# eltoto1219/vltk

Measured on AMD Instinct MI355X. Metric: images/sec FRCNN feature extraction, 800x1333 batch, higher is better.
Workload: dtype f16; 1 GPU; configs[1]: ResNet-101-C4 fp16 (the reference has no FPN: SURVEY.md D1), 32 synthetic 800x1333 images per GPU per step, R=300 RPN proposals through the Res5 head, max 100 detections/img, seeded synthetic weights; global_batch=32, parallelism=image-sharded x1, all-gather of output blocks

## Files before the change

include/vltk_hip.h:

```cpp
#ifndef VLTK_HIP_H
#define VLTK_HIP_H

#include <stddef.h>
#include <stdint.h>

#ifdef __cplusplus
extern "C" {
#endif

#define VK_OK 0
#define VK_EINVAL 1
#define VK_ENOTIMPL 2
#define VK_ENONFINITE 3
#define VK_EWEIGHTS 4
#define VK_EHIP 5
#define VK_ENOMEM 6

typedef enum { VK_F32 = 0, VK_F16 = 1, VK_I64 = 2, VK_I32 = 3, VK_BF16 = 4 } vk_dtype;
typedef enum { VK_ACT_NONE = 0, VK_ACT_RELU = 1, VK_ACT_GELU = 2 , VK_ACT_TANH = 3 } vk_act;

#define VK_MAX_ANCHOR_DIM 8
#define VK_MAX_NMS_THRESH 8

typedef struct vk_config {
// ... 139 lines not shown

size_t vk_packed_weight_bytes(int cout, int cin, int kh, int kw, int groups, vk_dtype dt);
int vk_packed_cout(int cout);
int vk_conv_slice_channels(int cin, int groups);
int vk_pack_conv_weight(const float *w_oihw_host, const float *bn_host, const float *bias_host,
                        int cout, int cin, int kh, int kw, int groups, vk_dtype dt,
                        void *w_packed_host, float *bias_packed_host);

int vk_conv2d(const void *x, int N, int H, int W, int cin,
              const void *w_packed, const float *bias_packed, const void *residual,
              void *y, int cout, int ldy, int kh, int kw, int stride, int pad, int dil, int groups,
              int relu, vk_dtype dt, vk_dtype out_dt, void *stream);

#define VK_ROUTE_GENERIC 0
#define VK_ROUTE_RING 1
#define VK_ROUTE_DUO 2
#define VK_ROUTE_WS 3
#define VK_ROUTE_GEMM4 4
#define VK_ROUTE_PANEL 5
#define VK_ROUTE_BLK 6
int vk_conv_route(int N, int H, int W, int cin, int cin2, int has_residual, int fused_mean, int cout, int ldy, int kh, int kw,
                  int stride, int pad, int dil, int groups, int relu, vk_dtype dt, vk_dtype out_dt);
int vk_panel_phase_images(int N, int H, int W, int dil);

int vk_conv1x1_dual(const void *x1, int cin1, const void *x2, int cin2, long M,
                    const void *w_packed, const float *bias_packed, const void *residual,
                    void *y, int cout, int relu, void *stream);

int vk_bottleneck64(const void *x, int N, int H, int W, int cin, int proj,
                    const void *w1_packed, const float *b1_packed, const void *w2_packed, const float *b2_packed,
                    const void *w3_packed, const float *b3_packed, void *y, void *stream);

int vk_fuse_shortcut(int cin, int cin_shortcut, int cout, int stride, vk_dtype dt);
int vk_bottleneck64_eligible(int cin, int cmid, int cout, int stride, int dil, int groups, int proj, int fused_shortcut,
                             long N, int H, int W, vk_dtype dt);

size_t vk_conv1x1_meanpool_workspace_bytes(int N, int HW, int cout);
int vk_conv1x1_meanpool(const void *x, int N, int HW, int cin, const void *w_packed, const float *bias_packed,
                        const void *residual, int cout, int relu, float *out_mean,
                        void *workspace, size_t workspace_bytes, void *stream);


int vk_linear(const void *x, long M, int K, const void *w_packed, const float *bias_packed, const void *residual,
              void *y, int N, int ldy, int act, vk_dtype dt, vk_dtype out_dt, void *stream);
int vk_layernorm(const void *x, int ldx, const float *gamma, const float *beta, void *y, int ldy, int M, int C,
                 float eps, float scale, int accumulate, vk_dtype dt, void *stream);
// ... 142 lines not shown
```

vltk_amd/_lib.py:

```python
import ctypes as C
import os

_HERE = os.path.dirname(os.path.abspath(__file__))
LIB_PATH = os.path.join(_HERE, "libvltk_hip.so")
if os.environ.get("VLTK_AMD_LIB"):
    LIB_PATH = os.environ["VLTK_AMD_LIB"]
elif os.environ.get("VLTK_AMD_ABLATION_LIB") == "1":
    LIB_PATH = LIB_PATH.replace("libvltk_hip.so", "libvltk_hip_ablation.so")

VK_OK, VK_EINVAL, VK_ENOTIMPL, VK_ENONFINITE, VK_EWEIGHTS, VK_EHIP, VK_ENOMEM = range(7)
VK_F32, VK_F16, VK_I64, VK_I32, VK_BF16 = 0, 1, 2, 3, 4
VK_ACT_NONE, VK_ACT_RELU, VK_ACT_GELU, VK_ACT_TANH = 0, 1, 2, 3
VK_ROUTE_GENERIC, VK_ROUTE_RING, VK_ROUTE_DUO, VK_ROUTE_WS, VK_ROUTE_GEMM4, VK_ROUTE_PANEL, VK_ROUTE_BLK = range(7)
VK_ATT_ROUTE_MFMA, VK_ATT_ROUTE_LDS, VK_ATT_ROUTE_TILED, VK_ATT_ROUTE_STREAM = range(4)
VK_MAX_ANCHOR_DIM = 8
VK_MAX_NMS_THRESH = 8
VK_MAX_IGNOREY = 64
VK_SELECT_CLASS_MAX, VK_SELECT_PER_CLASS, VK_SELECT_DETECTIONS = 0, 1, 2
VK_POOLER_ROIPOOL, VK_POOLER_ROIALIGN, VK_POOLER_ROIALIGNV2 = 0, 1, 2

_EXC = {
    VK_EINVAL: ValueError,
    VK_ENOTIMPL: NotImplementedError,
    VK_ENONFINITE: AssertionError,
# ... 67 lines not shown
                              C.POINTER(C.c_int64)]),
    "vk_forward_begin_ignorey": (_I, [_P, _P, _I, _I, _I, _P, _P, C.POINTER(vk_roi_params), C.POINTER(vk_outputs), _P,
                                      C.POINTER(C.c_int64), C.POINTER(vk_ignorey)]),
    "vk_forward_begin_select": (_I, [_P, _P, _I, _I, _I, _P, _P, C.POINTER(vk_select_params), C.POINTER(vk_outputs), _P,
                                     C.POINTER(C.c_int64), C.POINTER(vk_ignorey)]),
    "vk_forward_boxes_begin": (_I, [_P, _P, _I, _I, _I, _P, _P, _P, _I, _P, C.POINTER(vk_outputs), _P, C.POINTER(C.c_int64)]),
    "vk_forward_grid_begin": (_I, [_P, _P, _I, _I, _I, _P, _P, _I, _I, C.POINTER(vk_outputs), _P, C.POINTER(C.c_int64)]),
    "vk_grid_pool": (_I, [_P, _I, _I, _I, _I, _I, _P, _P, _I, _I, _I, _P, _I, _P, _P]),
    "vk_forward_end": (_I, [_P, C.c_int64]),
    "vk_given_boxes_ingest": (_I, [_P, _P, _P, _P, _I, _I, _P, _P, _P, _I, _I, _F, _I, _P, _P]),
    "vk_given_box_outputs": (_I, [_P, _P, _P, _P, _P, _P, _P, _P, _I, _I, _I, C.POINTER(vk_outputs), _P]),
    "vk_get_stage": (_I, [_P, C.c_char_p, C.POINTER(_P), C.POINTER(_I), C.POINTER(C.c_int64), C.POINTER(_I)]),
    "vk_memcpy_d2d": (_I, [_P, _P, _SZ, _P]),
    "vk_enable_stage_timing": (_I, [_P, _I]),
    "vk_get_stage_timing": (_I, [_P, C.POINTER(_F)]),
    "vk_enable_kernel_timing": (_I, [_P, _I]),
    "vk_get_kernel_timing": (_I, [_P, C.POINTER(C.c_int64), C.POINTER(_D), C.POINTER(_D), C.POINTER(_D), _I]),
    "vk_packed_weight_bytes": (_SZ, [_I, _I, _I, _I, _I, _I]),
    "vk_conv_slice_channels": (_I, [_I, _I]),
    "vk_packed_cout": (_I, [_I]),
    "vk_pack_conv_weight": (_I, [_P, _P, _P, _I, _I, _I, _I, _I, _I, _P, _P]),
    "vk_conv_route": (_I, [_I] * 18),
    "vk_panel_phase_images": (_I, [_I, _I, _I, _I]),
    "vk_conv1x1_dual": (_I, [_P, _I, _P, _I, C.c_long, _P, _P, _P, _P, _I, _I, _P]),
    "vk_bottleneck64": (_I, [_P, _I, _I, _I, _I, _I, _P, _P, _P, _P, _P, _P, _P, _P]),
    "vk_fuse_shortcut": (_I, [_I, _I, _I, _I, _I]),
    "vk_bottleneck64_eligible": (_I, [_I, _I, _I, _I, _I, _I, _I, _I, C.c_long, _I, _I, _I]),
    "vk_conv1x1_meanpool_workspace_bytes": (_SZ, [_I, _I, _I]),
    "vk_conv1x1_meanpool": (_I, [_P, _I, _I, _I, _P, _P, _P, _I, _I, _P, _P, _SZ, _P]),
    "vk_linear": (_I, [_P, C.c_long, _I, _P, _P, _P, _P, _I, _I, _I, _I, _I, _P]),
    "vk_layernorm": (_I, [_P, _I, _P, _P, _P, _I, _I, _I, _F, _F, _I, _I, _P]),
    "vk_embed_layernorm": (_I, [_P, _P, _I, _I, _P, _P, _P, _P, _P, _P, _I, _F, _I, _P]),
    "vk_attention": (_I, [_P, _I, _P, _I, _P, _I, _P, _P, _I, _I, _I, _I, _I, _I, _I, _P]),
    "vk_attention_tiled": (_I, [_P, _I, _P, _I, _P, _I, _P, _P, _I, _I, _I, _I, _I, _I, _I, _P]),
    "vk_attention_route": (_I, [_I] * 9),
    "vk_visualbert_embed": (_I, [_P, _P, _P, _P, _I, _I, _I, _I, _P, _I, _P, _I, _P, _P, _I, _P, _P, _I, _P, _P, _P, _I, _F, _I, _P]),
    "vk_vit_patchify": (_I, [_P, _I, _I, _I, _I, _I, _P, _I, _I, _P]),
    "vk_vit_assemble": (_I, [_P, _I, _P, _P, _I, _I, _P, _I, _I, _P]),
    "vk_roi_align": (_I, [_P, _P, _P, _P, _I, _I, _I, _P, _P, _I, _I, _I, _I, _P, _I, _P]),
    "vk_assign_levels": (_I, [_P, _I, _I, _I, _I, _F, _I, _P, _P]),
    "vk_upsample2x_add": (_I, [_P, _P, _P, _I, _I, _I, _I, _I, _I, _I, _P]),
    "vk_subsample2": (_I, [_P, _P, _I, _I, _I, _I, _I, _P]),
    "vk_relu_copy": (_I, [_P, _P, C.c_long, _I, _P]),
    "vk_rpn_multilevel_workspace_bytes": (_SZ, [_I, _I, _I, _I]),
    "vk_rpn_proposals_multilevel": (_I, [_P, _P, _P, _P, _I, _I, _P, _P, _I, _P, _P, _F, _P, _P, _F, _D, _I, _I, _P, _P, _P, _P, _P, _SZ, _P]),
    "vk_rpn_proposals_multilevel_ignorey": (_I, [_P, _P, _P, _P, _I, _I, _P, _P, _I, _P, _P, _F, _P, _P, _F, _D, _I, _I, _P, _P, _P, _P,
# ... 69 lines not shown
```

vltk_amd/csrc/conv3x3_panel.hip:

```cpp
#include <cstdio>
#include <type_traits>
#include <vector>

#include "vk_common.h"

namespace vk {

typedef _Float16 half8 __attribute__((ext_vector_type(8)));
typedef float floatx4 __attribute__((ext_vector_type(4)));
typedef _Float16 half4 __attribute__((ext_vector_type(4)));
typedef unsigned uintx4 __attribute__((ext_vector_type(4)));

struct PanelK {
    const char *x;
    const char *w;
    const float *bias;
    const char *res;
    char *y;
    int H, W, HW, M;
    int cin_bytes, ldy;
    int dil;
    int cstages;
    int wrow_bytes;
    int relu;
// ... 13 lines not shown
    const int W2 = p.W >> 1, Q = p.HW >> 2;
    const int ph = (gb >= Q ? 1 : 0) + (gb >= 2 * Q ? 1 : 0) + (gb >= 3 * Q ? 1 : 0);
    const int q = gb - ph * Q;
    const int qy = (int)(((unsigned)q * p.rcp_w2) >> 16), qx = q - qy * W2;
    return {qy, qx, (2 * qy + (ph >> 1)) * p.W + 2 * qx + (ph & 1)};
}

constexpr int P_NW = 6;
constexpr int P_WSLOT = 256 * 64;

#define VKP_GLDS16(gptr, lptr)                                                                         \
    __builtin_amdgcn_global_load_lds((const __attribute__((address_space(1))) void *)(gptr),          \
                                     (__attribute__((address_space(3))) void *)(lptr), 16, 0, 0)

template <int J, int PP>
constexpr int panel_in_window() {
    int c = 0;
    for (int d = 1; d <= P_NW - 2; ++d) {
        int t = ((J - d) % 9 + 9) % 9;
        if (t < PP) ++c;
    }
    return c;
}
template <int J>
constexpr int last_w_in_window() {
    int c = 0;
    for (int d = 1; d <= P_NW - 2; ++d) {
        int t = J - d;
        if (t < 0 || t + P_NW < 9) ++c;
    }
    return 2 * c;
}

template <int N>
__device__ __forceinline__ void vm_wait() {
    static_assert(N >= 0 && N <= 15, "vmcnt immediate");
    asm volatile("s_waitcnt vmcnt(%0)" ::"n"(N) : "memory");
}

template <int PP, int DBG, int TAG = 0, int MI = 8, int PHASE = 0>
__global__ __launch_bounds__(512, 2) void conv3x3_panel_kernel(PanelK p) {
    extern __shared__ __attribute__((aligned(16))) char smem[];
    static_assert(MI == 8 || MI == 9, "8 or 9 row tiles per wave");
    static_assert(!PHASE || (PP == 4 && MI == 8 && !(DBG & 9)), "the phase form: halo 128 = (W / 2 + 1) * 16 at W = 14, 256-row tiles");
    static_assert(MI == 8 || !(DBG & 8), "the LDS-staged epilogue is written for 128-row halves");
    constexpr int TILE = 2 * MI * 16;
    constexpr int PROWS = PP * 128;
    constexpr int HALO = (PROWS - TILE) / 2;
    constexpr int PBYTES = PROWS * 64;
    constexpr int WBASE = 2 * PBYTES;
    constexpr bool ZROW = PP == 3;
    constexpr int ZOFF = WBASE + P_NW * P_WSLOT;

    int bid = blockIdx.x;
    const int nwg = p.m_tiles * p.n_tiles;
    unsigned long st_k0 = 0;
    if constexpr (DBG & 4) asm volatile("s_memrealtime %0\n\ts_waitcnt lgkmcnt(0)" : "=s"(st_k0)::"memory");
    if constexpr (PP == 3 || PHASE) {
        if (p.tile_ctr && bid >= p.static_tiles) {
            int *mail = reinterpret_cast<int *>(smem + (PHASE ? 0 : 2 * PP * 128 * 64 + P_NW * P_WSLOT + 128));
            if (threadIdx.x == 0) {
                const unsigned v = atomicAdd(p.tile_ctr, 1u);
                if (v == p.ctr_last) *p.tile_ctr = 0u;
                *mail = p.static_tiles + (int)v;
            }
            __syncthreads();
            bid = __builtin_amdgcn_readfirstlane(*mail);
            if constexpr (PHASE) __syncthreads();
            if (bid >= nwg) return;
        }
    }
    const int q = nwg >> 3, r = nwg & 7, xcd = bid & 7;
    const int t_ = (xcd < r ? xcd * (q + 1) : r * (q + 1) + (xcd - r) * q) + (bid >> 3);
    const int n_tile = t_ % p.n_tiles, m_tile = t_ / p.n_tiles;
    const int m0 = m_tile * TILE, n0 = n_tile * 256;

    const int tid = threadIdx.x, lane = tid & 63;
    const int wave = __builtin_amdgcn_readfirstlane(tid >> 6);
    const int wr = wave >> 2, wc = wave & 3;
    const int g = lane >> 4, j = lane & 15;

    unsigned vm0 = 0, vm1 = 0, vm2 = 0;

    const int lrow = lane >> 2;
    const int lchunk = (lane & 3) ^ ((-(lrow >> 2)) & 3);
    const int pm_first = m0 - HALO + wave * 16 + lrow;
    const unsigned wsrc0 = (unsigned)(n0 + wave * 32 + lrow) * (unsigned)p.wrow_bytes + lchunk * 16;
    const unsigned wstep = 16u * p.wrow_bytes;
    int g0 = 0, gb0 = 0;
    if constexpr (PHASE) {
        g0 = (m0 >> 4) / p.HW;
        gb0 = (m0 >> 4) - g0 * p.HW;
    }
    auto blk_of = [&](int off, int &G) -> int {
        int t = gb0 + off;
        G = g0;
        while (t < 0) {
            t += p.HW;
            --G;
        }
        while (t >= p.HW) {
            t -= p.HW;
            ++G;
        }
        if (G < 0) G = 0, t = 0;
        if (G >= p.groups) G = p.groups - 1, t = p.HW - 1;
        return t;
    };
    [[maybe_unused]] unsigned ps_lane = 0, ps_blk[PP] = {};
    if constexpr (PHASE) {
// ... 2 lines not shown
        for (int q2 = 0; q2 < PP; ++q2) {
            int G;
            const int t = blk_of(wave - HALO / 16 + q2 * 8, G);
            ps_blk[q2] = __builtin_amdgcn_readfirstlane((unsigned)(G * 16 * p.HW + phase_blk(p, t).row) * (unsigned)p.cin_bytes);
        }
    }
    auto req_panel = [&](int cs, int piece) {
        if constexpr (PHASE) {
            unsigned pl = ps_lane;
            asm volatile("" : "+v"(pl));
            VKP_GLDS16(p.x + (pl + (ps_blk[piece] + cs * 64)), smem + (cs & 1) * PBYTES + (piece * 8 + wave) * 1024);
            return;
        }
        int pf = pm_first;
        asm volatile("" : "+v"(pf));
        const int m = min(max(pf + piece * 128, 0), p.M - 1);
        const unsigned off = (unsigned)m * (unsigned)p.cin_bytes + cs * 64 + lchunk * 16;
        VKP_GLDS16(p.x + off, smem + (cs & 1) * PBYTES + (piece * 8 + wave) * 1024);
    };
    auto req_w = [&](int slot, int cs, int tap, int i) {
        const unsigned koff = (unsigned)(tap * p.cstages + cs) * 64;
        unsigned wb_ = wsrc0;
        asm volatile("" : "+v"(wb_));
        VKP_GLDS16(p.w + (wb_ + i * wstep + koff), smem + WBASE + slot * P_WSLOT + (wave * 2 + i) * 1024);
    };

    const unsigned lds0 = (unsigned)(unsigned long)(__attribute__((address_space(3))) char *)smem;
    [[maybe_unused]] const unsigned zrow = lds0 + ZOFF;
    if constexpr (ZROW) {
        if (tid < 16) *reinterpret_cast<unsigned *>(smem + ZOFF + tid * 4) = 0u;
        asm volatile("s_waitcnt lgkmcnt(0)" ::: "memory");
    }
    unsigned w_a[2];
#pragma unroll
    for (int par = 0; par < 2; ++par) {
        const int wrow = wc * 64 + (j >> 2) * 8 + par * 4 + (j & 3);
        w_a[par] = lds0 + WBASE + wrow * 64 + ((g ^ ((-(wrow >> 2)) & 3)) << 4);
    }
    const int jbase = HALO + wr * (MI * 16) + j;
    auto x_addr_of = [&](int parity, int tap) -> unsigned {
        const int shift = PHASE ? ((tap / 3 - 1) * (p.W >> 1) + (tap % 3 - 1)) * 16 : ((tap / 3 - 1) * p.W + (tap % 3 - 1)) * p.dil;
        int jb = jbase;
        asm volatile("" : "+v"(jb));
        const int rb = jb + shift;
        return lds0 + parity * PBYTES + (rb << 6) + ((g ^ ((-(rb >> 2)) & 3)) << 4);
    };

// ... 52 lines not shown
        a0_ += so;                                      \
        a1_ += so;                                      \
        VKP_DSR(WF[0], a0_, 0);                         \
        VKP_DSR(WF[1], a1_, 0);                         \
        VKP_DSR(WF[2], a0_, 2048);                      \
        VKP_DSR(WF[3], a1_, 2048);                      \
    } while (0)

    auto tap_mask = [&](auto j_c) -> unsigned {
        constexpr int J = decltype(j_c)::value;
        unsigned tw = J < 3 ? vm0 : (J < 6 ? vm1 : vm2);
        if constexpr (PHASE)
            asm volatile("" : "+s"(tw));
        else
            asm volatile("" : "+v"(tw));
        return tw >> ((J % 3) * 9);
    };
    auto tap_word = [&](auto j_c) -> unsigned {
        constexpr int J = decltype(j_c)::value;
        unsigned tw = J < 3 ? vm0 : (J < 6 ? vm1 : vm2);
        asm volatile("" : "+v"(tw));
        return tw;
    };
    auto pre = [&](auto last_c, auto odd_c, auto j_c, unsigned xa, unsigned &xa_next, const half8 (&wcur)[4]) {
        constexpr bool LAST = decltype(last_c)::value;
        constexpr int ODD = decltype(odd_c)::value;
        constexpr int J = decltype(j_c)::value;
        const unsigned tm = ZROW ? 0u : tap_mask(j_c);
        [[maybe_unused]] const unsigned tw = ZROW ? tap_word(j_c) : 0u;
        constexpr bool has_next = !(LAST && J == 8);
        if constexpr (has_next) xa_next = (J == 8) ? x_addr_of(1 - ODD, 0) : x_addr_of(ODD, J + 1);
        VKP_DSRX(xw[3], xa, 3072, tw, J, 3); VKP_WAIT3(xw[0]); VKP_SB(); VKP_MMA_ROW(0, xw[0], wcur, tm); VKP_SB();
        VKP_DSRX(xw[0], xa, 4096, tw, J, 4); VKP_WAIT3(xw[1]); VKP_SB(); VKP_MMA_ROW(1, xw[1], wcur, tm); VKP_SB();
        VKP_DSRX(xw[1], xa, 5120, tw, J, 5); VKP_WAIT3(xw[2]); VKP_SB(); VKP_MMA_ROW(2, xw[2], wcur, tm); VKP_SB();
        VKP_DSRX(xw[2], xa, 6144, tw, J, 6); VKP_WAIT3(xw[3]); VKP_SB(); VKP_MMA_ROW(3, xw[3], wcur, tm); VKP_SB();
        if constexpr (MI == 9) {
            VKP_DSRX(xw[3], xa, 7168, tw, J, 7); VKP_DSRX(xw[4], xa, 8192, tw, J, 8); VKP_WAIT4(xw[0]); VKP_SB(); VKP_MMA_ROW(4, xw[0], wcur, tm); VKP_SB();
            asm volatile("s_waitcnt lgkmcnt(0)" : "+v"(xw[1]), "+v"(xw[2]), "+v"(xw[3]), "+v"(xw[MI == 9 ? 4 : 3])::"memory");
        } else {
            VKP_DSRX(xw[3], xa, 7168, tw, J, 7); VKP_WAIT3(xw[0]); VKP_SB(); VKP_MMA_ROW(4, xw[0], wcur, tm); VKP_SB();
            asm volatile("s_waitcnt lgkmcnt(0)" : "+v"(xw[1]), "+v"(xw[2]), "+v"(xw[3])::"memory");
        }
        VKP_SB();
        if constexpr (has_next) {
            constexpr int OUT = LAST ? last_w_in_window<J>() : 2 * (P_NW - 2) + panel_in_window<J, PP>();
            vm_wait<OUT>();
            if constexpr (!(DBG & 48) || ((DBG & 16) && J % 3 == 2)) asm volatile("s_barrier" ::: "memory");
        }
        VKP_SB();
    };
    auto post = [&](auto last_c, auto odd_c, auto j_c, int cs, unsigned xa_next, const half8 (&wcur)[4], half8 (&wnext)[4]) {
        constexpr bool LAST = decltype(last_c)::value;
        constexpr int ODD = decltype(odd_c)::value;
        constexpr int J = decltype(j_c)::value;
        static_assert(!(LAST && J == 8), "the final step has no POST");
        constexpr int SLOT = (3 * ODD + J) % P_NW;
        const unsigned tm = ZROW ? 0u : tap_mask(j_c);
        constexpr int JN = (J + 1) % 9;
        [[maybe_unused]] const unsigned twn = ZROW ? tap_word(std::integral_constant<int, JN>{}) : 0u;
        constexpr bool issue_w = !LAST || (J + P_NW < 9);
        constexpr bool issue_p = !LAST && (J < PP);
        constexpr unsigned so = (unsigned)((SLOT + 1) % P_NW) * P_WSLOT;
        VKP_READ_W(wnext, so);
        VKP_DSRX(xw[0], xa_next, 0, twn, JN, 0);
        VKP_SB();
        VKP_MMA_ROW(5, xw[1], wcur, tm);
        VKP_SB();
        if constexpr (issue_p) req_panel(cs + 1, J);
        if constexpr (issue_w) req_w(SLOT, cs + (J + P_NW) / 9, (J + P_NW) % 9, 0);
        VKP_DSRX(xw[1], xa_next, 1024, twn, JN, 1);
        VKP_SB();
        VKP_MMA_ROW(6, xw[2], wcur, tm);
        VKP_SB();
        if constexpr (issue_w) req_w(SLOT, cs + (J + P_NW) / 9, (J + P_NW) % 9, 1);
        VKP_DSRX(xw[2], xa_next, 2048, twn, JN, 2);
        VKP_SB();
        VKP_MMA_ROW(7, xw[3], wcur, tm);
        VKP_SB();
        if constexpr (MI == 9) {
            VKP_MMA_ROW(8, xw[MI == 9 ? 4 : 3], wcur, tm);
            VKP_SB();
        }
    };
    auto wset = [&](auto u_c) -> half8(&)[4] {
        if constexpr (decltype(u_c)::value % 2 == 0)
            return wa;
        else
            return wb;
    };
#define VKP_IC(V) std::integral_constant<int, (V)> {}
#define VKP_UNIT(LP, LC, U)                                                                                          \
    post(LP, VKP_IC(((U) - 1) / 9), VKP_IC(((U) - 1) % 9), cs + ((U) - 1) / 9, xan, wset(VKP_IC((U) - 1)), wset(VKP_IC(U)));  \
    xa = xan;                                                                                                        \
    pre(LC, VKP_IC((U) / 9), VKP_IC((U) % 9), xa, xan, wset(VKP_IC(U)));
    using T_ = std::integral_constant<bool, true>;
    using F_ = std::integral_constant<bool, false>;

#pragma unroll
    for (int q2 = 0; q2 < PP; ++q2) req_panel(0, q2);
#pragma unroll
    for (int st = 0; st < P_NW; ++st) {
        req_w(st, 0, st, 0);
        req_w(st, 0, st, 1);
    }
    if constexpr (PHASE) {
        unsigned u0 = 0, u1 = 0, u2 = 0;
#pragma unroll
        for (int mi = 0; mi < MI; ++mi) {
            int G;
            const PhaseBlk b = phase_blk(p, blk_of(wr * MI + mi, G));
            const unsigned c0 = b.qx >= 1, c2 = b.qx + 1 < (p.W >> 1);
            const unsigned cw = m0 + (wr * MI + mi) * 16 < p.M ? (c0 << mi) | (1u << (9 + mi)) | (c2 << (18 + mi)) : 0u;
            u0 |= b.qy >= 1 ? cw : 0u;
            u1 |= cw;
            u2 |= b.qy + 1 < (p.H >> 1) ? cw : 0u;
        }
        vm0 = __builtin_amdgcn_readfirstlane(u0);
        vm1 = __builtin_amdgcn_readfirstlane(u1);
        vm2 = __builtin_amdgcn_readfirstlane(u2);
    } else if (p.HW >= MI * 16 + p.W) {
        const int mbase = m0 + wr * (MI * 16);
        const int rem0 = mbase % p.HW, ho0 = rem0 / p.W, wo0 = rem0 - ho0 * p.W;
        const float rcpw = 1.0f / (float)p.W;
#pragma unroll
        for (int mi = 0; mi < MI; ++mi) {
            const int xcol = wo0 + mi * 16 + j;
// ... 17 lines not shown
    } else {
#pragma unroll
        for (int mi = 0; mi < MI; ++mi) {
            const int m = m0 + wr * (MI * 16) + mi * 16 + j;
            if (m < p.M) {
                const int n_img = m / p.HW;
                const int rem = m - n_img * p.HW;
                const int ho = rem / p.W, wo = rem - ho * p.W;
#pragma unroll
                for (int tap = 0; tap < 9; ++tap) {
                    const int hi = ho + (tap / 3 - 1) * p.dil, wi = wo + (tap % 3 - 1) * p.dil;
                    const unsigned ok = ((unsigned)hi < (unsigned)p.H && (unsigned)wi < (unsigned)p.W) ? 1u : 0u;
                    if (tap < 3)
                        vm0 |= ok << (tap * 9 + mi);
                    else if (tap < 6)
                        vm1 |= ok << ((tap - 3) * 9 + mi);
                    else
                        vm2 |= ok << ((tap - 6) * 9 + mi);
                }
            }
        }
    }

    vm_wait<2 * (P_NW - 1)>();
    asm volatile("s_barrier" ::: "memory");
    unsigned long st_c0 = 0, st_r0 = 0;
    if constexpr (DBG & 4) asm volatile("s_memtime %0\n\ts_memrealtime %1\n\ts_waitcnt lgkmcnt(0)" : "=s"(st_c0), "=s"(st_r0)::"memory");
    unsigned xa = x_addr_of(0, 0), xan = 0;
    VKP_READ_W(wa, 0u);
    {
        [[maybe_unused]] const unsigned tw0 = tap_word(VKP_IC(0));
        VKP_DSRX(xw[0], xa, 0, tw0, 0, 0);
        VKP_DSRX(xw[1], xa, 1024, tw0, 0, 1);
        VKP_DSRX(xw[2], xa, 2048, tw0, 0, 2);
    }
    pre(F_{}, VKP_IC(0), VKP_IC(0), xa, xan, wa);
    int cs = 0;
    for (; cs + 2 < CS; cs += 2) {
        VKP_UNIT(F_{}, F_{}, 1) VKP_UNIT(F_{}, F_{}, 2) VKP_UNIT(F_{}, F_{}, 3) VKP_UNIT(F_{}, F_{}, 4) VKP_UNIT(F_{}, F_{}, 5)
        VKP_UNIT(F_{}, F_{}, 6) VKP_UNIT(F_{}, F_{}, 7) VKP_UNIT(F_{}, F_{}, 8) VKP_UNIT(F_{}, F_{}, 9) VKP_UNIT(F_{}, F_{}, 10)
        VKP_UNIT(F_{}, F_{}, 11) VKP_UNIT(F_{}, F_{}, 12) VKP_UNIT(F_{}, F_{}, 13) VKP_UNIT(F_{}, F_{}, 14) VKP_UNIT(F_{}, F_{}, 15)
        VKP_UNIT(F_{}, F_{}, 16) VKP_UNIT(F_{}, F_{}, 17)
        post(F_{}, VKP_IC(1), VKP_IC(8), cs + 1, xan, wb, wa);
        xa = xan;
        pre(F_{}, VKP_IC(0), VKP_IC(0), xa, xan, wa);
    }
    VKP_UNIT(F_{}, F_{}, 1) VKP_UNIT(F_{}, F_{}, 2) VKP_UNIT(F_{}, F_{}, 3) VKP_UNIT(F_{}, F_{}, 4) VKP_UNIT(F_{}, F_{}, 5)
    VKP_UNIT(F_{}, F_{}, 6) VKP_UNIT(F_{}, F_{}, 7) VKP_UNIT(F_{}, F_{}, 8) VKP_UNIT(F_{}, T_{}, 9) VKP_UNIT(T_{}, T_{}, 10)
    VKP_UNIT(T_{}, T_{}, 11) VKP_UNIT(T_{}, T_{}, 12) VKP_UNIT(T_{}, T_{}, 13) VKP_UNIT(T_{}, T_{}, 14) VKP_UNIT(T_{}, T_{}, 15)
    VKP_UNIT(T_{}, T_{}, 16) VKP_UNIT(T_{}, T_{}, 17)
    {
        const unsigned tm = ZROW ? 0u : tap_mask(VKP_IC(8));
        VKP_MMA_ROW(5, xw[1], wb, tm);
        VKP_MMA_ROW(6, xw[2], wb, tm);
        VKP_MMA_ROW(7, xw[3], wb, tm);
        if constexpr (MI == 9) VKP_MMA_ROW(8, xw[MI == 9 ? 4 : 3], wb, tm);
    }
    unsigned long st_c1 = 0, st_r1 = 0;
    if constexpr (DBG & 4) asm volatile("s_memtime %0\n\ts_memrealtime %1\n\ts_waitcnt lgkmcnt(0)" : "=s"(st_c1), "=s"(st_r1)::"memory");
#undef VKP_UNIT
#undef VKP_IC
#undef VKP_DSR
#undef VKP_DSRX
#undef VKP_WAIT3
#undef VKP_WAIT4
#undef VKP_MMA_ROW
#undef VKP_READ_W
#undef VKP_SB
// ... 151 lines not shown
    const long n8 = ((M + 255) / 256 * nt + n_cu - 1) / n_cu, n9 = ((M + 287) / 288 * nt + n_cu - 1) / n_cu;
    if (n8 > 4) return 9;
    return n9 * 9 < n8 * 8 ? 9 : 8;
}

bool conv3x3_panel_eligible(const ConvArgs &a) {
    const char *v = getenv("VK_CONV3X3_PANEL");
    if (v && v[0] == '0') return false;
    if (a.stem || a.dt != VK_F16 || a.out_dt != VK_F16 || a.relu > 1) return false;
    if (a.kh != 3 || a.kw != 3 || a.stride != 1 || a.pad != a.dil) return false;
    if (a.Cout % 256 != 0 || a.ldy != a.Cout || a.Cin % 64 != 0 || a.Cin < 128) return false;
    if (panel_pp(a) == 0) return false;
    if ((long)a.N * a.H * a.W * a.Cin * 2 >= (1L << 32)) return false;
    return true;
}

int conv3x3_panel_phase_images(const ConvArgs &a) {
    const char *v = getenv("VK_PANEL_PHASE");
    if (v && v[0] == '0') return 0;
    if (a.dil != 2 || a.H % 2 != 0 || a.W % 2 != 0 || a.W > 14 || a.H > 1024 || a.N < 16) return 0;
    return a.N / 16 * 16;
}

static int launch_panel_one(const ConvArgs &a, hipStream_t stream, bool phase);

int launch_conv3x3_panel(const ConvArgs &a, hipStream_t stream) {
    const int np = conv3x3_panel_phase_images(a);
    if (np == 0) return launch_panel_one(a, stream, false);
    ConvArgs b = a;
    b.N = np;
    VK_TRY(launch_panel_one(b, stream, true));
    if (np == a.N) return VK_OK;
    const size_t rows = (size_t)np * a.H * a.W;
    b.N = a.N - np;
    b.x = (const char *)a.x + rows * a.Cin * 2;
    b.y = (char *)a.y + rows * a.ldy * 2;
    if (a.res) b.res = (const char *)a.res + rows * a.ldy * 2;
    return launch_panel_one(b, stream, false);
}

static int launch_panel_one(const ConvArgs &a, hipStream_t stream, bool phase) {
    DeviceState *ds = nullptr;
    VK_TRY(device_state(&ds));
    PanelK k;
    k.x = (const char *)a.x;
    k.w = (const char *)a.w;
    k.bias = a.bias;
    k.res = (const char *)a.res;
    k.y = (char *)a.y;
    k.H = a.H;
    k.W = a.W;
    k.HW = a.H * a.W;
    const long M = (long)a.N * a.H * a.W;
    VK_REQUIRE(M > 0 && M < (1L << 31) - 512, VK_EINVAL, "conv3x3_panel: M=%ld out of range", M);
    VK_REQUIRE(M * a.Cin * 2 < (1L << 32) && (long)a.Cout * 9 * a.Cin * 2 < (1L << 32), VK_EINVAL,
               "conv3x3_panel: tensor beyond the 32-bit DMA offsets (M=%ld Cin=%d Cout=%d)", M, a.Cin, a.Cout);
    k.M = (int)M;
    k.cin_bytes = a.Cin * 2;
    k.ldy = a.ldy;
    k.dil = a.dil;
    k.cstages = a.Cin / 32;
    k.wrow_bytes = 9 * a.Cin * 2;
    k.relu = a.relu;
    const int mi = phase ? 8 : panel_mi(a, M, ds->n_cu), pp = phase ? 4 : panel_pp(a, mi);
    k.groups = phase ? a.N / 16 : 0;
    k.rcp_w2 = phase ? 65536u / (unsigned)(a.W / 2) + 1u : 0u;
    k.m_tiles = ceil_div(k.M, mi * 32);
    k.n_tiles = a.Cout / 256;
    Timed t;
    VK_TRY(t.begin(stream));
    const int total_tiles = k.m_tiles * k.n_tiles;
    k.tile_ctr = nullptr;
    k.static_tiles = total_tiles;
    int n_wgs = total_tiles;
    const char *dyn_env = getenv("VK_PANEL_DYNAMIC");
    const bool dyn_off = dyn_env && dyn_env[0] == '0';
    if (!dyn_off && (pp == 3 || phase) && total_tiles >= 16 * 256) {
        VK_TRY(acquire_tile_counter(&k.tile_ctr));
        k.static_tiles = total_tiles * 15 / 16 / 8 * 8;
        n_wgs = total_tiles + (total_tiles / 32 + 63) / 64 * 64;
        k.ctr_last = (unsigned)(n_wgs - k.static_tiles - 1);
    }
    const dim3 grid(n_wgs), block(512);
#ifdef VK_ABLATION
    const int dbg = getenv("VK_CONV256_DBG") ? atoi(getenv("VK_CONV256_DBG")) : 0;
#endif
    const int smem = 2 * pp * 128 * 64 + P_NW * P_WSLOT + (pp == 3 ? 256 : 0);
    k.stamps = nullptr;
#define VKP_LAUNCH(PP_, DBG_, TAG_, MI_)                                                                                                   \
    do {                                                                                                                                   \
        VK_TRY(set_max_lds(conv3x3_panel_kernel<PP_, DBG_, TAG_, MI_>, 2 * PP_ * 128 * 64 + P_NW * P_WSLOT + (PP_ == 3 ? 256 : 0)));        \
        hipLaunchKernelGGL((conv3x3_panel_kernel<PP_, DBG_, TAG_, MI_>), grid, block, smem, stream, k);                                     \
    } while (0)
#ifdef VK_ABLATION
    if (const char *sf = getenv("VK_PANEL_STAMPS"); sf && pp == 3) {
        const size_t nb = (size_t)grid.x * 6 * sizeof(unsigned long);
        VK_CHECK_HIP(hipMalloc((void **)&k.stamps, nb));
        VK_CHECK_HIP(hipMemset(k.stamps, 0, nb));
        if (mi == 9)
            VKP_LAUNCH(3, 4, 0, 9);
        else
            VKP_LAUNCH(3, 4, 0, 8);
        VK_CHECK_HIP(hipStreamSynchronize(stream));
        std::vector<unsigned long> h((size_t)grid.x * 6);
        VK_CHECK_HIP(hipMemcpy(h.data(), k.stamps, nb, hipMemcpyDeviceToHost));
        VK_CHECK_HIP(hipFree(k.stamps));
        if (FILE *f = fopen(sf, "a")) {
            fprintf(f, "# wg k_loop_cycles k_loop_ticks workgroup_ticks ticks_before_k_loop start_tick end_tick (tick = 10 ns)\n");
            for (unsigned w = 0; w < grid.x; ++w)
                fprintf(f, "%u %lu %lu %lu %lu %lu %lu\n", w, h[(size_t)w * 6], h[(size_t)w * 6 + 1], h[(size_t)w * 6 + 2], h[(size_t)w * 6 + 3], h[(size_t)w * 6 + 4],
                        h[(size_t)w * 6 + 5]);
            fclose(f);
        }
    } else if (mi == 8 && pp == 3 && dbg == 8)
        VKP_LAUNCH(3, 8, 0, 8);
    else if (mi == 8 && pp == 3 && dbg == 1)
        VKP_LAUNCH(3, 1, 0, 8);
    else if (mi == 9 && pp == 3 && dbg == 1)
        VKP_LAUNCH(3, 1, 0, 9);
    else if (mi == 9 && pp == 3 && dbg == 16)
        VKP_LAUNCH(3, 16, 0, 9);
    else if (mi == 9 && pp == 3 && dbg == 32)
        VKP_LAUNCH(3, 32, 0, 9);
    else
#endif
#ifdef VK_ABLATION
    if (const char *pv = getenv("VK_PANEL_PHASE"); phase && pv && pv[0] == 'A') {
        VK_TRY(set_max_lds(conv3x3_panel_kernel<4, 0, 0, 8, 1>, smem));
        hipLaunchKernelGGL((conv3x3_panel_kernel<4, 0, 0, 8, 1>), grid, block, smem, stream, k);
    } else
#endif
    if (phase) {
        VK_TRY(set_max_lds(conv3x3_panel_kernel<4, 0, 0, 8, 2>, smem));
        hipLaunchKernelGGL((conv3x3_panel_kernel<4, 0, 0, 8, 2>), grid, block, smem, stream, k);
    } else if (mi == 8 && pp == 3 && a.concurrent)
        VKP_LAUNCH(3, 0, 1, 8);
    else if (mi == 8 && pp == 3)
        VKP_LAUNCH(3, 0, 0, 8);
    else if (mi == 8 && a.concurrent)
        VKP_LAUNCH(4, 0, 1, 8);
    else if (mi == 8)
        VKP_LAUNCH(4, 0, 0, 8);
    else if (pp == 3 && a.concurrent)
        VKP_LAUNCH(3, 0, 1, 9);
    else if (pp == 3)
        VKP_LAUNCH(3, 0, 0, 9);
    else if (a.concurrent)
        VKP_LAUNCH(4, 0, 1, 9);
    else
        VKP_LAUNCH(4, 0, 0, 9);
#undef VKP_LAUNCH
    VK_CHECK_HIP(hipGetLastError());
    return t.end(stream, a.concurrent ? 6 : 4, 2.0 * (double)k.M * a.Cout * 9 * a.Cin, k.M, a.Cout, a.Cin, 9, 1,
                 2.0 * ((double)k.M * a.Cin + (double)k.M * a.Cout * (a.res ? 2 : 1) + (double)a.Cout * 9 * a.Cin));
}
// ... 3 lines not shown
```

vltk_amd/csrc/stage_api.hip:

```cpp
#include <algorithm>
#include <cmath>
#include <cstdlib>

#include "vk_common.h"

using namespace vk;

namespace vk {

void fill_conv_args(ConvArgs &a, int N, int H, int W, int cin, int cout, int ldy, int k, int stride, int pad, int dil, int groups,
                    int relu, vk_dtype dt, vk_dtype out_dt) {
    memset(&a, 0, sizeof(a));
    a.N = N;
    a.H = H;
    a.W = W;
    a.Cin = cin;
    conv_out_hw(H, W, k, stride, pad, dil, &a.Ho, &a.Wo);
    a.Cout = cout;
    a.ldy = ldy;
    a.kh = a.kw = k;
    a.stride = stride;
    a.pad = pad;
    a.dil = dil;
    a.groups = groups;
// ... 161 lines not shown
        return -VK_EINVAL;
    }
    static const char here = 0;
    ConvArgs a;
    fill_conv_args(a, N, H, W, cin, cout, ldy, kh, stride, pad, dil, groups, relu, dt, out_dt);
    if (!(a.Ho > 0 && a.Wo > 0 && N > 0)) {
        set_error("conv_route: empty output");
        return -VK_EINVAL;
    }
    a.x = a.w = &here;
    a.res = has_residual ? &here : nullptr;
    a.x2 = cin2 > 0 ? &here : nullptr;
    a.Cin2 = cin2;
    a.pool_part = fused_mean ? (float *)&here : nullptr;
    return conv_route_checked(a);
}

int vk_panel_phase_images(int N, int H, int W, int dil) {
    ConvArgs a;
    fill_conv_args(a, N, H, W, 128, 256, 256, 3, 1, dil, dil, 1, 0, VK_F16, VK_F16);
    return conv3x3_panel_phase_images(a);
}

int vk_conv1x1_dual(const void *x1, int cin1, const void *x2, int cin2, long M, const void *w_packed, const float *bias_packed,
                    const void *residual, void *y, int cout, int relu, void *stream) {
    VK_REQUIRE(x1 && x2 && M > 0 && M < (1L << 31), VK_EINVAL, "conv1x1_dual: bad arguments");
    ConvArgs a;
    fill_conv_args(a, 1, 1, (int)M, cin1, cout, cout, 1, 1, 0, 1, 1, relu, VK_F16, VK_F16);
    a.x = x1;
    a.x2 = x2;
    a.Cin2 = cin2;
    a.w = w_packed;
    a.bias = bias_packed;
    a.res = residual;
    a.y = y;
    return launch_conv(a, (hipStream_t)stream);
}

int vk_conv1x1_rows(const void *x1, int cin1, const void *x2, int cin2, long M, const int32_t *m_dev, const int32_t *x2_idx,
                    const void *w_packed, const float *bias_packed, void *y, int cout, int relu, void *stream) {
    VK_REQUIRE(x1 && w_packed && bias_packed && y && M > 0 && M < (1L << 31), VK_EINVAL, "conv1x1_rows: bad arguments");
    VK_REQUIRE(!x2_idx || x2, VK_EINVAL, "conv1x1_rows: a row index needs a second input");
    ConvArgs a;
    fill_conv_args(a, 1, 1, (int)M, cin1, cout, cout, 1, 1, 0, 1, 1, relu, VK_F16, VK_F16);
    a.x = x1;
    a.x2 = x2;
// ... 241 lines not shown
```

vltk_amd/csrc/vk_common.h:

```cpp
#pragma once
#include <hip/hip_runtime.h>

#include <atomic>
#include <cstdarg>
#include <cstdint>
#include <cstdio>
#include <cstring>
#include <vector>

#include "vltk_hip.h"

namespace vk {

void set_error(const char *fmt, ...);

#define VK_CHECK_HIP(expr)                                                                    \
    do {                                                                                      \
        hipError_t _e = (expr);                                                               \
        if (_e != hipSuccess) {                                                               \
            vk::set_error("%s:%d: %s -> %s", __FILE__, __LINE__, #expr, hipGetErrorString(_e)); \
            return VK_EHIP;                                                                   \
        }                                                                                     \
    } while (0)

// ... 39 lines not shown
    void *y;
    int N, H, W, Cin;
    int Ho, Wo, Cout, ldy;
    int kh, kw, stride, pad, dil;
    int groups;
    int concurrent;
    float *pool_part;
    const void *x2;
    int Cin2;
    int relu;
    int stem;
    const int32_t *m_dev;
    const int32_t *x2_idx;
    vk_dtype dt, out_dt;
};
int launch_conv(const ConvArgs &a, hipStream_t stream);
int conv_route(const ConvArgs &a);
int conv_route_checked(const ConvArgs &a);
bool conv256_eligible(const ConvArgs &a);
int launch_conv256(const ConvArgs &a, hipStream_t stream);
bool conv3x3_panel_eligible(const ConvArgs &a);
int launch_conv3x3_panel(const ConvArgs &a, hipStream_t stream);
int conv3x3_panel_phase_images(const ConvArgs &a);
bool conv_gemm4_eligible(const ConvArgs &a);
int launch_conv_gemm4(const ConvArgs &a, hipStream_t stream);
int acquire_tile_counter(unsigned **ctr);
bool conv256_dual_ok(const ConvArgs &a);
bool conv_duo_eligible(const ConvArgs &a);
int launch_conv_duo(const ConvArgs &a, hipStream_t stream);
bool conv_ws_eligible(const ConvArgs &a);
int launch_conv_ws(const ConvArgs &a, hipStream_t stream);
bool conv3x3_blk_eligible(const ConvArgs &a);
int launch_conv3x3_blk(const ConvArgs &a, hipStream_t stream);
bool bneck_fused_eligible(int cin, int cmid, int cout, int stride, int groups, bool proj, long N, int H, int W, vk_dtype dt);
int launch_bneck_fused(const void *x, int N, int H, int W, int cin, bool proj, const void *w1, const float *b1, const void *w2,
                       const float *b2, const void *w3, const float *b3, void *y, bool concurrent, hipStream_t stream);
bool conv_duo_dual_ok(const ConvArgs &a);
bool conv_duo_pool_ok(const ConvArgs &a);
size_t conv_duo_pool_part_bytes(long M, int Cout);
bool conv_pool_sums_f64(long N, int HW, int Cin, int Cout, bool dual);
bool conv_ws_pool_ok(const ConvArgs &a);
int launch_pool_finish(const float *part, int N, int HoWo, int Cin, int Cout, bool dual, float *out, hipStream_t stream);

struct KernelTimer {
    struct Rec {
        int bucket;
// ... 210 lines not shown
```

Baseline: 520.1 images/sec.

## Use 512x128 tall tiles with 4x2 wave layout in phase-form panel conv

```diff
diff --git a/include/vltk_hip.h b/include/vltk_hip.h
--- a/include/vltk_hip.h
+++ b/include/vltk_hip.h
@@ -185,6 +185,7 @@
 int vk_conv_route(int N, int H, int W, int cin, int cin2, int has_residual, int fused_mean, int cout, int ldy, int kh, int kw,
                   int stride, int pad, int dil, int groups, int relu, vk_dtype dt, vk_dtype out_dt);
 int vk_panel_phase_images(int N, int H, int W, int dil);
+int vk_panel_phase_tile_rows(int N, int H, int W, int dil, int cout);
 
 int vk_conv1x1_dual(const void *x1, int cin1, const void *x2, int cin2, long M,
                     const void *w_packed, const float *bias_packed, const void *residual,
diff --git a/vltk_amd/_lib.py b/vltk_amd/_lib.py
--- a/vltk_amd/_lib.py
+++ b/vltk_amd/_lib.py
@@ -113,6 +113,7 @@
     "vk_pack_conv_weight": (_I, [_P, _P, _P, _I, _I, _I, _I, _I, _I, _P, _P]),
     "vk_conv_route": (_I, [_I] * 18),
     "vk_panel_phase_images": (_I, [_I, _I, _I, _I]),
+    "vk_panel_phase_tile_rows": (_I, [_I, _I, _I, _I, _I]),
     "vk_conv1x1_dual": (_I, [_P, _I, _P, _I, C.c_long, _P, _P, _P, _P, _I, _I, _P]),
     "vk_bottleneck64": (_I, [_P, _I, _I, _I, _I, _I, _P, _P, _P, _P, _P, _P, _P, _P]),
     "vk_fuse_shortcut": (_I, [_I, _I, _I, _I, _I]),
diff --git a/vltk_amd/csrc/conv3x3_panel.hip b/vltk_amd/csrc/conv3x3_panel.hip
--- a/vltk_amd/csrc/conv3x3_panel.hip
+++ b/vltk_amd/csrc/conv3x3_panel.hip
@@ -59,14 +59,23 @@
     }
     return c;
 }
-template <int J>
-constexpr int last_w_in_window() {
+template <int J, int PP, int NWP, bool FIRST>
+constexpr int pieces_in_window() {
+    static_assert(PP <= 6, "a panel piece of the previous stage in the window of a tap other than 0");
+    if (FIRST) return NWP * (P_NW - 2);
+    const int c = NWP * (P_NW - 2) + panel_in_window<J, PP>();
+    const int after_panel = NWP * (9 - PP);
+    return J == 8 && after_panel < c ? after_panel : c;
+}
+template <int J, int PP, int NWP>
+constexpr int last_in_window() {
     int c = 0;
     for (int d = 1; d <= P_NW - 2; ++d) {
         int t = J - d;
-        if (t < 0 || t + P_NW < 9) ++c;
-    }
-    return 2 * c;
+        if (t < 0 || t + P_NW < 9) c += NWP;
+        if (t < 0 && 9 + t < PP) ++c;
+    }
+    return c;
 }
 
 template <int N>
@@ -75,19 +84,26 @@
     asm volatile("s_waitcnt vmcnt(%0)" ::"n"(N) : "memory");
 }
 
-template <int PP, int DBG, int TAG = 0, int MI = 8, int PHASE = 0>
+template <int PP, int DBG, int TAG = 0, int MI = 8, int PHASE = 0, int WR = 2>
 __global__ __launch_bounds__(512, 2) void conv3x3_panel_kernel(PanelK p) {
     extern __shared__ __attribute__((aligned(16))) char smem[];
     static_assert(MI == 8 || MI == 9, "8 or 9 row tiles per wave");
-    static_assert(!PHASE || (PP == 4 && MI == 8 && !(DBG & 9)), "the phase form: halo 128 = (W / 2 + 1) * 16 at W = 14, 256-row tiles");
+    static_assert(WR == 2 || WR == 4, "2 x 4 or 4 x 2 waves");
+    static_assert(!PHASE || (PP == (WR == 4 ? 6 : 4) && MI == 8 && !(DBG & 9)), "the phase form: halo 128 = (W / 2 + 1) * 16 at W = 14, 256- or 512-row tiles");
+    static_assert(WR == 2 || PHASE == 2, "512 x 128 tiles: the phase form only (a plain res4 launch would read its panel twice)");
     static_assert(MI == 8 || !(DBG & 8), "the LDS-staged epilogue is written for 128-row halves");
-    constexpr int TILE = 2 * MI * 16;
+    constexpr int WC = 8 / WR;
+    constexpr int CT = 64 * WC;
+    constexpr int NWP = CT / 128;
+    constexpr int WSLOT = CT * 64;
+    constexpr int TILE = WR * MI * 16;
     constexpr int PROWS = PP * 128;
     constexpr int HALO = (PROWS - TILE) / 2;
     constexpr int PBYTES = PROWS * 64;
     constexpr int WBASE = 2 * PBYTES;
+    static_assert(HALO >= (PHASE ? 128 : 48) && WBASE + P_NW * WSLOT + (PP == 3 || WR == 4 ? 256 : 0) <= 160 * 1024, "halo / LDS");
     constexpr bool ZROW = PP == 3;
-    constexpr int ZOFF = WBASE + P_NW * P_WSLOT;
+    constexpr int ZOFF = WBASE + P_NW * WSLOT;
 
     int bid = blockIdx.x;
     const int nwg = p.m_tiles * p.n_tiles;
@@ -95,7 +111,8 @@
     if constexpr (DBG & 4) asm volatile("s_memrealtime %0\n\ts_waitcnt lgkmcnt(0)" : "=s"(st_k0)::"memory");
     if constexpr (PP == 3 || PHASE) {
         if (p.tile_ctr && bid >= p.static_tiles) {
-            int *mail = reinterpret_cast<int *>(smem + (PHASE ? 0 : 2 * PP * 128 * 64 + P_NW * P_WSLOT + 128));
+            constexpr bool MAIL_IN_PANEL = PHASE && WR == 2;
+            int *mail = reinterpret_cast<int *>(smem + (MAIL_IN_PANEL ? 0 : ZOFF + 128));
             if (threadIdx.x == 0) {
                 const unsigned v = atomicAdd(p.tile_ctr, 1u);
                 if (v == p.ctr_last) *p.tile_ctr = 0u;
@@ -103,18 +120,18 @@
             }
             __syncthreads();
             bid = __builtin_amdgcn_readfirstlane(*mail);
-            if constexpr (PHASE) __syncthreads();
+            if constexpr (MAIL_IN_PANEL) __syncthreads();
             if (bid >= nwg) return;
         }
     }
     const int q = nwg >> 3, r = nwg & 7, xcd = bid & 7;
     const int t_ = (xcd < r ? xcd * (q + 1) : r * (q + 1) + (xcd - r) * q) + (bid >> 3);
     const int n_tile = t_ % p.n_tiles, m_tile = t_ / p.n_tiles;
-    const int m0 = m_tile * TILE, n0 = n_tile * 256;
+    const int m0 = m_tile * TILE, n0 = n_tile * CT;
 
     const int tid = threadIdx.x, lane = tid & 63;
     const int wave = __builtin_amdgcn_readfirstlane(tid >> 6);
-    const int wr = wave >> 2, wc = wave & 3;
+    const int wr = wave / WC, wc = wave & (WC - 1);
     const int g = lane >> 4, j = lane & 15;
 
     unsigned vm0 = 0, vm1 = 0, vm2 = 0;
@@ -122,7 +139,7 @@
     const int lrow = lane >> 2;
     const int lchunk = (lane & 3) ^ ((-(lrow >> 2)) & 3);
     const int pm_first = m0 - HALO + wave * 16 + lrow;
-    const unsigned wsrc0 = (unsigned)(n0 + wave * 32 + lrow) * (unsigned)p.wrow_bytes + lchunk * 16;
+    const unsigned wsrc0 = (unsigned)(n0 + wave * (16 * NWP) + lrow) * (unsigned)p.wrow_bytes + lchunk * 16;
     const unsigned wstep = 16u * p.wrow_bytes;
     int g0 = 0, gb0 = 0;
     if constexpr (PHASE) {
@@ -171,7 +188,7 @@
         const unsigned koff = (unsigned)(tap * p.cstages + cs) * 64;
         unsigned wb_ = wsrc0;
         asm volatile("" : "+v"(wb_));
-        VKP_GLDS16(p.w + (wb_ + i * wstep + koff), smem + WBASE + slot * P_WSLOT + (wave * 2 + i) * 1024);
+        VKP_GLDS16(p.w + (wb_ + i * wstep + koff), smem + WBASE + slot * WSLOT + (wave * NWP + i) * 1024);
     };
 
     const unsigned lds0 = (unsigned)(unsigned long)(__attribute__((address_space(3))) char *)smem;
@@ -270,8 +287,8 @@
         asm volatile("" : "+v"(tw));
         return tw;
     };
-    auto pre = [&](auto last_c, auto odd_c, auto j_c, unsigned xa, unsigned &xa_next, const half8 (&wcur)[4]) {
-        constexpr bool LAST = decltype(last_c)::value;
+    auto pre = [&](auto last_c, auto odd_c, auto j_c, unsigned xa, unsigned &xa_next, const half8 (&wcur)[4], auto first_c) {
+        constexpr bool LAST = decltype(last_c)::value, FIRST = decltype(first_c)::value;
         constexpr int ODD = decltype(odd_c)::value;
         constexpr int J = decltype(j_c)::value;
         const unsigned tm = ZROW ? 0u : tap_mask(j_c);
@@ -291,7 +308,7 @@
         }
         VKP_SB();
         if constexpr (has_next) {
-            constexpr int OUT = LAST ? last_w_in_window<J>() : 2 * (P_NW - 2) + panel_in_window<J, PP>();
+            constexpr int OUT = LAST ? last_in_window<J, PP, NWP>() : pieces_in_window<J, PP, NWP, FIRST>();
             vm_wait<OUT>();
             if constexpr (!(DBG & 48) || ((DBG & 16) && J % 3 == 2)) asm volatile("s_barrier" ::: "memory");
         }
@@ -308,7 +325,7 @@
         [[maybe_unused]] const unsigned twn = ZROW ? tap_word(std::integral_constant<int, JN>{}) : 0u;
         constexpr bool issue_w = !LAST || (J + P_NW < 9);
         constexpr bool issue_p = !LAST && (J < PP);
-        constexpr unsigned so = (unsigned)((SLOT + 1) % P_NW) * P_WSLOT;
+        constexpr unsigned so = (unsigned)((SLOT + 1) % P_NW) * WSLOT;
         VKP_READ_W(wnext, so);
         VKP_DSRX(xw[0], xa_next, 0, twn, JN, 0);
         VKP_SB();
@@ -320,7 +337,7 @@
         VKP_SB();
         VKP_MMA_ROW(6, xw[2], wcur, tm);
         VKP_SB();
-        if constexpr (issue_w) req_w(SLOT, cs + (J + P_NW) / 9, (J + P_NW) % 9, 1);
+        if constexpr (issue_w && NWP == 2) req_w(SLOT, cs + (J + P_NW) / 9, (J + P_NW) % 9, 1);
         VKP_DSRX(xw[2], xa_next, 2048, twn, JN, 2);
         VKP_SB();
         VKP_MMA_ROW(7, xw[3], wcur, tm);
@@ -340,7 +357,7 @@
 #define VKP_UNIT(LP, LC, U)                                                                                          \
     post(LP, VKP_IC(((U) - 1) / 9), VKP_IC(((U) - 1) % 9), cs + ((U) - 1) / 9, xan, wset(VKP_IC((U) - 1)), wset(VKP_IC(U)));  \
     xa = xan;                                                                                                        \
-    pre(LC, VKP_IC((U) / 9), VKP_IC((U) % 9), xa, xan, wset(VKP_IC(U)));
+    pre(LC, VKP_IC((U) / 9), VKP_IC((U) % 9), xa, xan, wset(VKP_IC(U)), F_{});
     using T_ = std::integral_constant<bool, true>;
     using F_ = std::integral_constant<bool, false>;
 
@@ -349,7 +366,7 @@
 #pragma unroll
     for (int st = 0; st < P_NW; ++st) {
         req_w(st, 0, st, 0);
-        req_w(st, 0, st, 1);
+        if constexpr (NWP == 2) req_w(st, 0, st, 1);
     }
     if constexpr (PHASE) {
         unsigned u0 = 0, u1 = 0, u2 = 0;
@@ -413,7 +430,7 @@
         }
     }
 
-    vm_wait<2 * (P_NW - 1)>();
+    vm_wait<NWP * (P_NW - 1)>();
     asm volatile("s_barrier" ::: "memory");
     unsigned long st_c0 = 0, st_r0 = 0;
     if constexpr (DBG & 4) asm volatile("s_memtime %0\n\ts_memrealtime %1\n\ts_waitcnt lgkmcnt(0)" : "=s"(st_c0), "=s"(st_r0)::"memory");
@@ -425,7 +442,7 @@
         VKP_DSRX(xw[1], xa, 1024, tw0, 0, 1);
         VKP_DSRX(xw[2], xa, 2048, tw0, 0, 2);
     }
-    pre(F_{}, VKP_IC(0), VKP_IC(0), xa, xan, wa);
+    pre(F_{}, VKP_IC(0), VKP_IC(0), xa, xan, wa, T_{});
     int cs = 0;
     for (; cs + 2 < CS; cs += 2) {
         VKP_UNIT(F_{}, F_{}, 1) VKP_UNIT(F_{}, F_{}, 2) VKP_UNIT(F_{}, F_{}, 3) VKP_UNIT(F_{}, F_{}, 4) VKP_UNIT(F_{}, F_{}, 5)
@@ -434,7 +451,7 @@
         VKP_UNIT(F_{}, F_{}, 16) VKP_UNIT(F_{}, F_{}, 17)
         post(F_{}, VKP_IC(1), VKP_IC(8), cs + 1, xan, wb, wa);
         xa = xan;
-        pre(F_{}, VKP_IC(0), VKP_IC(0), xa, xan, wa);
+        pre(F_{}, VKP_IC(0), VKP_IC(0), xa, xan, wa, F_{});
     }
     VKP_UNIT(F_{}, F_{}, 1) VKP_UNIT(F_{}, F_{}, 2) VKP_UNIT(F_{}, F_{}, 3) VKP_UNIT(F_{}, F_{}, 4) VKP_UNIT(F_{}, F_{}, 5)
     VKP_UNIT(F_{}, F_{}, 6) VKP_UNIT(F_{}, F_{}, 7) VKP_UNIT(F_{}, F_{}, 8) VKP_UNIT(F_{}, T_{}, 9) VKP_UNIT(T_{}, T_{}, 10)
@@ -632,6 +649,12 @@
     return a.N / 16 * 16;
 }
 
+int conv3x3_panel_phase_tile_rows(const ConvArgs &a) {
+    if (a.Cout % 256 != 0 || conv3x3_panel_phase_images(a) == 0) return 0;
+    const char *v = getenv("VK_PANEL_TALL");
+    return v && v[0] == '0' ? 256 : 512;
+}
+
 static int launch_panel_one(const ConvArgs &a, hipStream_t stream, bool phase);
 
 int launch_conv3x3_panel(const ConvArgs &a, hipStream_t stream) {
@@ -672,11 +695,16 @@
     k.cstages = a.Cin / 32;
     k.wrow_bytes = 9 * a.Cin * 2;
     k.relu = a.relu;
-    const int mi = phase ? 8 : panel_mi(a, M, ds->n_cu), pp = phase ? 4 : panel_pp(a, mi);
+    bool tall = phase && conv3x3_panel_phase_tile_rows(a) == 512;
+#ifdef VK_ABLATION
+    if (const char *pv = getenv("VK_PANEL_PHASE"); pv && pv[0] == 'A') tall = false;
+#endif
+    const int mi = phase ? 8 : panel_mi(a, M, ds->n_cu), pp = tall ? 6 : (phase ? 4 : panel_pp(a, mi));
+    const int wslot = tall ? P_WSLOT / 2 : P_WSLOT;
     k.groups = phase ? a.N / 16 : 0;
     k.rcp_w2 = phase ? 65536u / (unsigned)(a.W / 2) + 1u : 0u;
-    k.m_tiles = ceil_div(k.M, mi * 32);
-    k.n_tiles = a.Cout / 256;
+    k.m_tiles = ceil_div(k.M, tall ? 512 : mi * 32);
+    k.n_tiles = a.Cout / (tall ? 128 : 256);
     Timed t;
     VK_TRY(t.begin(stream));
     const int total_tiles = k.m_tiles * k.n_tiles;
@@ -695,7 +723,7 @@
 #ifdef VK_ABLATION
     const int dbg = getenv("VK_CONV256_DBG") ? atoi(getenv("VK_CONV256_DBG")) : 0;
 #endif
-    const int smem = 2 * pp * 128 * 64 + P_NW * P_WSLOT + (pp == 3 ? 256 : 0);
+    const int smem = 2 * pp * 128 * 64 + P_NW * wslot + (pp == 3 || tall ? 256 : 0);
     k.stamps = nullptr;
 #define VKP_LAUNCH(PP_, DBG_, TAG_, MI_)                                                                                                   \
     do {                                                                                                                                   \
@@ -740,7 +768,10 @@
         hipLaunchKernelGGL((conv3x3_panel_kernel<4, 0, 0, 8, 1>), grid, block, smem, stream, k);
     } else
 #endif
-    if (phase) {
+    if (tall) {
+        VK_TRY(set_max_lds(conv3x3_panel_kernel<6, 0, 0, 8, 2, 4>, smem));
+        hipLaunchKernelGGL((conv3x3_panel_kernel<6, 0, 0, 8, 2, 4>), grid, block, smem, stream, k);
+    } else if (phase) {
         VK_TRY(set_max_lds(conv3x3_panel_kernel<4, 0, 0, 8, 2>, smem));
         hipLaunchKernelGGL((conv3x3_panel_kernel<4, 0, 0, 8, 2>), grid, block, smem, stream, k);
     } else if (mi == 8 && pp == 3 && a.concurrent)
diff --git a/vltk_amd/csrc/stage_api.hip b/vltk_amd/csrc/stage_api.hip
--- a/vltk_amd/csrc/stage_api.hip
+++ b/vltk_amd/csrc/stage_api.hip
@@ -207,6 +207,12 @@
     return conv3x3_panel_phase_images(a);
 }
 
+int vk_panel_phase_tile_rows(int N, int H, int W, int dil, int cout) {
+    ConvArgs a;
+    fill_conv_args(a, N, H, W, 128, cout, cout, 3, 1, dil, dil, 1, 0, VK_F16, VK_F16);
+    return conv3x3_panel_phase_tile_rows(a);
+}
+
 int vk_conv1x1_dual(const void *x1, int cin1, const void *x2, int cin2, long M, const void *w_packed, const float *bias_packed,
                     const void *residual, void *y, int cout, int relu, void *stream) {
     VK_REQUIRE(x1 && x2 && M > 0 && M < (1L << 31), VK_EINVAL, "conv1x1_dual: bad arguments");
diff --git a/vltk_amd/csrc/vk_common.h b/vltk_amd/csrc/vk_common.h
--- a/vltk_amd/csrc/vk_common.h
+++ b/vltk_amd/csrc/vk_common.h
@@ -85,6 +85,7 @@
 bool conv3x3_panel_eligible(const ConvArgs &a);
 int launch_conv3x3_panel(const ConvArgs &a, hipStream_t stream);
 int conv3x3_panel_phase_images(const ConvArgs &a);
+int conv3x3_panel_phase_tile_rows(const ConvArgs &a);
 bool conv_gemm4_eligible(const ConvArgs &a);
 int launch_conv_gemm4(const ConvArgs &a, hipStream_t stream);
 int acquire_tile_counter(unsigned **ctr);
```

New measurement: 530.2 images/sec, median of 6. 1.9% higher.
